# better-flow/better-flow

Measured on AMD Instinct MI355X. Metric: Mevents/s motion-compensated (warp→converged score), 1M-ev slice, 1/2/4/8 GPU, higher is better.
Workload: dtype f64

## Files before the change

better_flow_amd/csrc/bf_device_fns.h:

```cpp
#pragma once
#include <hip/hip_runtime.h>
#include <limits.h>

#include "bf_device.h"
#include "bf_kernels.h"
#include "../../include/bf_flow_color.h"
#include <math.h>
#include <math.h>

namespace bf {

__device__ __forceinline__ int trunc_x86(double v) { return bf_double_to_int_x86(v); }

__device__ __forceinline__ int trunc_scatter(double v) { return (v == v) ? __double2int_rz(v) : INT_MIN; }

__device__ __forceinline__ bool valid_px(float p) { return p > 1e-6f; }

__device__ __forceinline__ double div_10000(double x) {
    constexpr double R = 1.0 / 10000.0;
    const double q0 = x * R;
    const double r = fma(-q0, 10000.0, x);
    return fma(r, R, q0);
}
__device__ __forceinline__ float div_127(float x) {
    constexpr float R = 1.0f / 127.0f;
    const float q0 = x * R;
    const float r = fmaf(-q0, 127.0f, x);
    return fmaf(r, R, q0);
}

__device__ __forceinline__ double div_1e9(double x) {
    constexpr double R = 1.0 / 1000000000.0;
    const double q0 = x * R;
    const double r = fma(-q0, 1000000000.0, x);
    return fma(r, R, q0);
}

__device__ __forceinline__ double2 uv_from_n(double2 v) {
    const double len = hypot(v.x, v.y);
    const double speed = len / (127.0 / (double)(1000000000 / (1 * 10000)));
    double2 o;
    o.x = (len == 0) ? 0 : speed * v.x / len;
    o.y = (len == 0) ? 0 : speed * v.y / len;
    return o;
}

__device__ __forceinline__ double2 uv_from_n_nz(double2 v, double nz) {
    const double len = hypot(v.x, v.y);
    const double speed = len / (nz / (double)(1000000000 / (1 * 10000)));
    double2 o;
    o.x = (len == 0) ? 0 : speed * v.x / len;
    o.y = (len == 0) ? 0 : speed * v.y / len;
    return o;
}

__device__ __forceinline__ double pr_from_p(uint32_t fr, float prod) {
    return (double)fr - div_10000((double)prod);
}

__device__ __forceinline__ void warp_products(const WarpParams& wp, double pr_x, double pr_y, int32_t t, float2& q,
                                              double& nx, double& ny) {
    const double rx = pr_x - wp.cx, ry = pr_y - wp.cy;
    const double qx = wp.c * rx - wp.s * ry;
    const double qy = wp.s * rx + wp.c * ry;
    nx = ((-qx) * wp.div + (qx - rx)) + wp.dnx;
    ny = ((-qy) * wp.div + (qy - ry)) + wp.dny;
    const float kx = div_127((float)nx);
    const float ky = div_127((float)ny);
    const float ft = (float)t;
    q.x = kx * ft;
    q.y = ky * ft;
}

__device__ __forceinline__ int assign_pixel(const WarpParams& wp, uint32_t v, int32_t t, int scale, int x_sh, int y_sh, int wsx,
                                            int wsy, int C) {
    const uint32_t fx = v & 0xffffu, fy = v >> 16;
    float2 q;
    double nx, ny;
    warp_products(wp, (double)fx, (double)fy, t, q, nx, ny);
    const int X = trunc_scatter(pr_from_p(fx, q.x) * (double)scale + (double)x_sh);
    const int Y = trunc_scatter(pr_from_p(fy, q.y) * (double)scale + (double)y_sh);
    const int hs = scale / 2;
    if ((X >= wsx + hs) || (X < hs) || (Y >= wsy + hs) || (Y < hs)) return -1;
    return X * C + Y;
}

template <class T>
__device__ __forceinline__ T sload(const T* p) {
    static_assert(sizeof(T) % 4 == 0, "whole words");
    typedef const __attribute__((address_space(4))) uint32_t* cptr;
    const cptr src = reinterpret_cast<cptr>(reinterpret_cast<uintptr_t>(p));
    T out;
    uint32_t* dst = reinterpret_cast<uint32_t*>(&out);
#pragma unroll
    for (int i = 0; i < (int)(sizeof(T) / 4); ++i) dst[i] = src[i];
    return out;
}

__device__ __forceinline__ int wave_min(int v) {
    for (int o = 32; o > 0; o >>= 1) v = min(v, __shfl_down(v, o, 64));
    return v;
}
__device__ __forceinline__ int wave_max(int v) {
    for (int o = 32; o > 0; o >>= 1) v = max(v, __shfl_down(v, o, 64));
    return v;
}
__device__ __forceinline__ long long wave_sum(long long v) {
    for (int o = 32; o > 0; o >>= 1) v += __shfl_down(v, o, 64);
    return v;
}
__device__ __forceinline__ double wave_sum(double v) {
    for (int o = 32; o > 0; o >>= 1) v += __shfl_down(v, o, 64);
    return v;
}
__device__ __forceinline__ unsigned long long wave_sum_u64(unsigned long long v) {
    for (int o = 32; o > 0; o >>= 1) v += __shfl_down(v, o, 64);
    return v;
}
__device__ __forceinline__ uint32_t wave_max_u32(uint32_t v) {
    for (int o = 32; o > 0; o >>= 1) v = max(v, (uint32_t)__shfl_down(v, o, 64));
    return v;
}
__device__ __forceinline__ unsigned long long wave_max_u64(unsigned long long v) {
    for (int o = 32; o > 0; o >>= 1) {
        const unsigned long long w = (unsigned long long)__shfl_down((long long)v, o, 64);
        v = w > v ? w : v;
    }
    return v;
}

template <class F>
__device__ __forceinline__ void for_each_wave_key(int key, F&& f) {
    unsigned long long pending = __ballot(key >= 0);
    while (pending) {
        const int k0 = __shfl(key, __ffsll((long long)pending) - 1, 64);
        const unsigned long long same = __ballot(key == k0);
        f(k0, same);
        pending &= ~same;
    }
}

constexpr int kBoxTR = 32, kBoxTC = 64;
template <int MAXH>
__device__ __forceinline__ void box_sum_tile(const uint32_t* __restrict__ src, uint32_t* __restrict__ dst, int R, int C, int hs,
                                             int tr0, int tc0) {
    __shared__ uint32_t s_in[(kBoxTR + 2 * MAXH) * (kBoxTC + 2 * MAXH)];
    __shared__ uint32_t s_row[(kBoxTR + 2 * MAXH) * kBoxTC];
    const int IR = kBoxTR + 2 * hs, IC = kBoxTC + 2 * hs;
    for (int idx = threadIdx.x; idx < IR * IC; idx += kThreads) {
        const int lr = idx / IC, lc = idx - lr * IC;
        const int gr = tr0 - hs + lr, gc = tc0 - hs + lc;
        s_in[idx] = (gr >= 0 && gr < R && gc >= 0 && gc < C) ? src[(size_t)gr * C + gc] : 0u;
    }
    __syncthreads();
    for (int idx = threadIdx.x; idx < IR * kBoxTC; idx += kThreads) {
        const int lr = idx / kBoxTC, lc = idx % kBoxTC;
        uint32_t sum = 0;
        for (int d = 0; d <= 2 * hs; ++d) sum += s_in[lr * IC + lc + d];
        s_row[idx] = sum;
    }
    __syncthreads();
    for (int idx = threadIdx.x; idx < kBoxTR * kBoxTC; idx += kThreads) {
        const int lr = idx / kBoxTC, lc = idx % kBoxTC;
        const int gr = tr0 + lr, gc = tc0 + lc;
        if (gr >= R || gc >= C) continue;
        uint32_t sum = 0;
        for (int d = 0; d <= 2 * hs; ++d) sum += s_row[(lr + d) * kBoxTC + lc];
        dst[(size_t)gr * C + gc] = sum;
    }
}

__device__ __forceinline__ int row_bin(int row, const BinGrid& g) { return (int)__umulhi((uint32_t)row, g.mul_r); }

constexpr int kTicketGroups = 32;

constexpr int kTlLaunches = 64;
__device__ __forceinline__ void tl_stamp(unsigned long long* tl, int launch, int slot) {
#ifdef BF_TIMELINE
    if (!tl || launch >= kTlLaunches || threadIdx.x != 0) return;
// ... 662 lines not shown
```

better_flow_amd/csrc/bf_scatter.hip:

```cpp
#include <atomic>
#include <hip/hip_runtime.h>
#include <hip/hip_ext.h>
#include <limits.h>
#include <cstdlib>

#include "bf_device.h"
#include "bf_device_fns.h"
#include "bf_kernels.h"

namespace bf {

template <class T>
__device__ __forceinline__ T ld_idx(const T* base, uint32_t idx) {
    return *reinterpret_cast<const T*>(reinterpret_cast<const char*>(base) + idx * (uint32_t)sizeof(T));
}

constexpr int kMaxTileRows = 192;

struct ScatterGeo {
    int X0, Y0, L, LR;
    int zw;
};
template <bool WARP>
__device__ __forceinline__ bool event_target(const ScatterHot& hs, float2* p, uint32_t i, uint32_t v, int32_t ti,
                                             double pr_x, double pr_y, int& X, int& Y) {
    const uint32_t fx = v & 0xffffu, fy = v >> 16;
    if (WARP) {
        float2 q;
        double nx, ny;
        warp_products(hs.wp, pr_x, pr_y, ti, q, nx, ny);
        __hip_atomic_store(reinterpret_cast<unsigned long long*>(reinterpret_cast<char*>(p) + i * 8u),
                           ((unsigned long long)__float_as_uint(q.y) << 32) | (unsigned long long)__float_as_uint(q.x),
                           __ATOMIC_RELAXED, __HIP_MEMORY_SCOPE_AGENT);
        pr_x = pr_from_p(fx, q.x);
        pr_y = pr_from_p(fy, q.y);
    }
    const int s = hs.scale, hsc = hs.scale / 2;
    if (hsc > 0) {
        X = __double2int_rz(pr_x * (double)s + (double)hs.x_sh);
        Y = __double2int_rz(pr_y * (double)s + (double)hs.y_sh);
    } else {
        X = trunc_scatter(pr_x * (double)s + (double)hs.x_sh);
        Y = trunc_scatter(pr_y * (double)s + (double)hs.y_sh);
    }
    return (unsigned)(X - hsc) < (unsigned)hs.wsx && (unsigned)(Y - hsc) < (unsigned)hs.wsy;
}
__device__ __forceinline__ void overflow_add(const ScatterHot& hs, const BinScatterArgs& a, int X, int Y, unsigned long long dt) {
    const size_t kk = (size_t)X * (size_t)hs.C + (size_t)Y;
    atomicAdd(&a.ovf_plane[kk], dt);
    atomicAdd(&a.ovf_cplane[kk], 1u);
    atomicOr(&a.ovf_bits[(size_t)X * (size_t)a.ovf_pitch + (size_t)(Y >> 5) + 1], 1u << (Y & 31));
}

template <bool WARP>
__device__ __forceinline__ void scatter_event(const ScatterHot& hs, const ScatterGeo& sg, unsigned long long* s_tile,
                                              const BinScatterArgs& a, float2* p, uint32_t i, uint32_t v, int32_t ti,
                                              double pr_x, double pr_y, uint32_t& n_ovf) {
    int X, Y;
    if (!event_target<WARP>(hs, p, i, v, ti, pr_x, pr_y, X, Y)) return;
    const unsigned long long dt = (unsigned long long)((long long)ti - hs.tmin);
    const int lx = X - sg.X0, ly = Y - sg.Y0;
    if (hs.bin_ok && (unsigned)lx < (unsigned)sg.LR && (unsigned)ly < (unsigned)sg.L) {
        atomicAdd(&s_tile[__mul24(lx, sg.L) + ly], (1ull << hs.bin_tbits) + dt);
    } else {
        overflow_add(hs, a, X, Y, dt);
        ++n_ovf;
    }
}

constexpr uint32_t kNoEntry = 0xffffffffu;
template <bool WARP>
__device__ __forceinline__ uint32_t list_event(const ScatterHot& hs, const ScatterGeo& sg, const BinScatterArgs& a, float2* p,
                                               uint32_t i, uint32_t v, int32_t ti, double pr_x, double pr_y, bool take_overflow,
                                               int& row, uint32_t& n_ovf) {
    int X, Y;
    row = 0;
    if (!event_target<WARP>(hs, p, i, v, ti, pr_x, pr_y, X, Y)) return kNoEntry;
    const int lx = X - sg.X0, ly = Y - sg.Y0;
    if (hs.bin_ok && (unsigned)lx < (unsigned)sg.LR && (unsigned)ly < (unsigned)sg.L) {
        row = lx + (sg.zw ? (ly < sg.zw ? 0 : (ly >= sg.L - sg.zw ? 2 * sg.LR : sg.LR)) : 0);
        return (uint32_t)(__mul24(lx, sg.L) + ly);
    }
    if (take_overflow) {
        overflow_add(hs, a, X, Y, (unsigned long long)((long long)ti - hs.tmin));
        ++n_ovf;
    }
    return kNoEntry;
}
__device__ __forceinline__ void list_row_scan(uint32_t* s_row, int LR, uint32_t* crow, int lane) {
    uint32_t carry = 0;
    for (int r0 = 0; r0 < LR; r0 += 64) {
        const int r = r0 + lane;
        const uint32_t v = r < LR ? s_row[1 + r] : 0u;
        uint32_t incl = v;
#pragma unroll
        for (int o = 1; o < 64; o <<= 1) {
            const uint32_t u = __shfl_up(incl, o, 64);
            if (lane >= o) incl += u;
        }
        if (r < LR) {
            s_row[1 + r] = carry + incl - v;
            crow[r] = carry + incl - v;
        }
        carry += (uint32_t)__builtin_amdgcn_readlane((int)incl, 63);
    }
    if (lane == 0) crow[LR] = carry;
}
__device__ __forceinline__ void list_put(const ScatterHot& hs, const ScatterGeo& sg, const BinScatterArgs& a, uint32_t* s_row,
                                         uint32_t code, int row, int32_t ti, uint32_t LL, unsigned long long* vals,
                                         uint16_t* cidx, uint32_t& n_ovf) {
    const unsigned long long dt = (unsigned long long)((long long)ti - hs.tmin);
    const uint32_t slot = atomicAdd(&s_row[1 + row], 1u);
    if (slot < LL) {
        vals[slot] = (1ull << hs.bin_tbits) + dt;
        cidx[slot] = (uint16_t)code;
    } else {
        const int lx = row >= 2 * sg.LR ? row - 2 * sg.LR : (row >= sg.LR ? row - sg.LR : row);
        overflow_add(hs, a, sg.X0 + lx, sg.Y0 + (int)code - __mul24(lx, sg.L), dt);
        ++n_ovf;
    }
}

template <int THREADS>
__device__ __forceinline__ void flush_tile(const unsigned long long* s_tile, unsigned long long* slab, int LL, int tid) {
    const bf_u32x4* src4 = reinterpret_cast<const bf_u32x4*>(s_tile);
    for (int i = tid; i < LL / 2; i += THREADS) {
        const bf_u32x4 v = src4[i];
        asm volatile("global_store_dwordx4 %0, %1, off sc1" :: "v"(slab + 2 * i), "v"(v) : "memory");
    }
}
__device__ __forceinline__ uint32_t margin_preload(const BinScatterArgs& a, int b, uint32_t n_prev, int tid) {
    return (uint32_t)tid < n_prev ? a.mlist[(size_t)b * (size_t)a.mcap + tid] : 0xffffffffu;
}
__device__ __forceinline__ void margin_clear(const BinScatterArgs& a, int b, uint32_t n_prev, uint32_t e0, int tid, int threads) {
    if (e0 != 0xffffffffu) a.m_prev[e0] = 0ull;
    const uint32_t* lst = a.mlist + (size_t)b * (size_t)a.mcap;
    for (uint32_t i = tid + threads; i < n_prev; i += threads) a.m_prev[lst[i]] = 0ull;
}
template <int THREADS>
__device__ __forceinline__ void flush_split(const unsigned long long* s_tile, const BinScatterArgs& a, int b, int X0, int Y0, int C,
                                            uint32_t* s_mcnt , int tid) {
    const BinGrid& g = a.g;
    const bf_u32x4* src4 = reinterpret_cast<const bf_u32x4*>(s_tile);
    const int half = g.L >> 1, hD = g.D >> 1, lgh = g.lg - 1;
    unsigned long long* own = a.slabs + (size_t)b * (size_t)(g.TS * g.TSR);
    const int nown = g.TSR << lgh;
    for (int i = tid; i < nown; i += THREADS) {
        const int r = i >> lgh, q = i - (r << lgh);
        const bf_u32x4 v = src4[(r + g.D) * half + hD + q];
        asm volatile("global_store_dwordx4 %0, %1, off sc1" :: "v"(own + 2 * i), "v"(v) : "memory");
    }
    uint32_t* lst = a.mlist + (size_t)b * (size_t)a.mcap;
    const int nfull = 2 * g.D * half, nmar = nfull + g.TSR * g.D;
    const int lgD = 31 - __clz(g.D);
    for (int j = tid; j < nmar; j += THREADS) {
        int lx, lp;
        if (j < nfull) {
            const int r = (int)__umulhi((uint32_t)j, g.mul_h);
            lp = j - r * half;
            lx = r < g.D ? r : r + g.TSR;
        } else {
            const int k = j - nfull, r = k >> lgD, q = k & (g.D - 1);
            lx = g.D + r;
            lp = q < hD ? q : q + (g.TS >> 1);
        }
        const bf_u32x4 v = src4[lx * half + lp];
        const unsigned long long w0 = ((unsigned long long)v.y << 32) | v.x, w1 = ((unsigned long long)v.w << 32) | v.z;
        if (w0 | w1) {
            const uint32_t px = (uint32_t)((X0 + lx) * C + Y0 + 2 * lp);
            if (w0) {
                __hip_atomic_fetch_add(&a.m_cur[px], w0, __ATOMIC_RELAXED, __HIP_MEMORY_SCOPE_AGENT);
                lst[atomicAdd(&s_mcnt[0], 1u)] = px;
            }
            if (w1) {
                __hip_atomic_fetch_add(&a.m_cur[px + 1], w1, __ATOMIC_RELAXED, __HIP_MEMORY_SCOPE_AGENT);
                lst[atomicAdd(&s_mcnt[0], 1u)] = px + 1;
            }
        }
    }
    uint32_t arrived = 0;
    if ((tid & 63) == 0) arrived = atomicAdd(&s_mcnt[1], 1u);
    arrived = (uint32_t)__builtin_amdgcn_readfirstlane((int)arrived);
    if (arrived == THREADS / 64 - 1 && (tid & 63) == 0) a.mcount[b] = s_mcnt[0];
}
__global__ __launch_bounds__(256) void k_margin_clean(unsigned long long* mplane, const uint32_t* mlist, uint32_t* mcount, int mcap) {
    const int b = blockIdx.x;
    const uint32_t n = mcount[b];
    const uint32_t* lst = mlist + (size_t)b * (size_t)mcap;
    for (uint32_t i = threadIdx.x; i < n; i += 256) mplane[lst[i]] = 0ull;
    __syncthreads();
    if (threadIdx.x == 0) mcount[b] = 0u;
}
void launch_margin_clean(unsigned long long* mplane, const uint32_t* mlist, uint32_t* mcount, int nbins, int mcap, hipStream_t s) {
    if (nbins > 0) hipLaunchKernelGGL(k_margin_clean, dim3(nbins), dim3(256), 0, s, mplane, mlist, mcount, mcap);
}

template <bool WARP, int THREADS, int U, int FMT>
__global__ __launch_bounds__(THREADS) void k_bin_warp_scatter(const uint32_t* __restrict__ pre_bin_start, const DevState* pre_st_in,
                                                              MomentAcc* pre_acc, BinScatterArgs a) {
    constexpr bool COMPACT = FMT == 2;
    constexpr bool SPLIT = FMT == 3;
// ... 117 lines not shown
        store_state();
        if (tid < 64) list_row_scan(s_row, (g.zw ? 3 : 1) * LR, a.chdr + (size_t)b * (size_t)((g.zw ? 3 : 1) * LR + 1), tid);
        __syncthreads();
        unsigned long long* vals = a.slabs + (size_t)b * (size_t)LL;
        uint16_t* cidx = a.cidx + (size_t)b * (size_t)LL;
        if (single) {
#pragma unroll
            for (int k = 0; k < U; ++k)
                if (code[k] != kNoEntry) list_put(hs, sg, a, s_row, code[k], row[k], vt[k], (uint32_t)LL, vals, cidx, n_ovf);
        } else {
            for (base = beg; base < end; base += THREADS * U) {
                load_pass();
                previous_positions();
#pragma unroll
                for (int k = 0; k < U; ++k) {
                    const uint32_t i = base + k * THREADS + tid;
                    if (i >= end) continue;
                    int r;
                    const uint32_t cd = list_event<false>(hs, sg, a, p, i, vxy[k], vt[k], ppx[k], ppy[k], false, r, n_ovf);
                    if (cd != kNoEntry) list_put(hs, sg, a, s_row, cd, r, vt[k], (uint32_t)LL, vals, cidx, n_ovf);
                }
            }
        }
        if (n_ovf) { atomicAdd(ovf_counter(a.ovf_cur, b), n_ovf); a.ovf_cur[0] = 1u; }
        tl_stamp(a.tl, a.j, 4);
        return;
    }
    for (;;) {
#pragma unroll
        for (int k = 0; k < U; ++k) {
            const uint32_t i = base + k * THREADS + tid;
            if (i >= end) continue;
            scatter_event<WARP>(hs, sg, s_tile, a, p, i, vxy[k], vt[k], ppx[k], ppy[k], n_ovf);
        }
        base += THREADS * U;
        if (base >= end) break;
        load_pass();
        previous_positions();
    }
    if (n_ovf) { atomicAdd(ovf_counter(a.ovf_cur, b), n_ovf); a.ovf_cur[0] = 1u; }
    if (SPLIT) margin_clear(a, b, m_prev_n, m_e0, tid, THREADS);
    tl_stamp(a.tl, a.j, 2);
    __syncthreads();
    tl_stamp(a.tl, a.j, 3);
    store_state();
    if (SPLIT) flush_split<THREADS>(s_tile, a, b, X0, Y0, hs.C, s_mcnt, tid);
    else flush_tile<THREADS>(s_tile, a.slabs + (size_t)b * (size_t)LL, LL, tid);
    tl_stamp(a.tl, a.j, 4);
}

template <bool WARP, int THREADS, int U, int FMT>
__global__ __launch_bounds__(THREADS) void k_bin_warp_scatter_lean(const uint32_t* __restrict__ pre_bin_start, const DevState* pre_st_in,
                                                                   MomentAcc* , BinScatterArgs a) {
    constexpr bool COMPACT = FMT == 2;
    constexpr bool SPLIT = FMT == 3;
    extern __shared__ unsigned long long s_tile[];
    __shared__ uint32_t s_row[FMT == 2 ? 1 + 3 * kMaxTileRows : 1];
    __shared__ uint32_t s_mcnt[2];
    if (FMT == 2)
        for (int r = threadIdx.x; r <= 3 * kMaxTileRows; r += THREADS) s_row[r] = 0;
    if (SPLIT && threadIdx.x < 2) s_mcnt[threadIdx.x] = 0;
    const BinGrid& g = a.g;
    const int L = g.L, LR = g.LR, LL = g.LR * g.L;
    const int b = blockIdx.x, tid = threadIdx.x;
    const uint32_t beg = sload(pre_bin_start + b), end = sload(pre_bin_start + b + 1);
    const HotState h0 = sload(&pre_st_in->hot);
    const uint32_t m_prev_n = SPLIT ? sload(a.mcount + b) : 0u;
    const int X0 = (b / g.nbc) * g.TSR - g.D, Y0 = (b - (b / g.nbc) * g.nbc) * g.TS - g.D;
    if (!COMPACT) {
        ulonglong2* z = reinterpret_cast<ulonglong2*>(s_tile);
        for (int i = tid; i < LL / 2; i += THREADS) z[i] = make_ulonglong2(0ull, 0ull);
    }
    if (h0.done) {
        if (b == 0 && tid < kStateWords) {
            const unsigned long long state_word = reinterpret_cast<const unsigned long long*>(a.st_in)[tid];
            reinterpret_cast<unsigned long long*>(a.st_out)[tid] = state_word;
            if (a.snap) reinterpret_cast<unsigned long long*>(a.snap)[tid] = state_word;
        }
        return;
    }
    ScatterHot hs;
    hs.done = h0.done; hs.bin_tbits = h0.bin_tbits; hs.bin_ok = h0.bin_ok; hs.fmt = h0.fmt; hs.scale = h0.scale; hs.C = h0.C;
    hs.wsx = h0.wsx; hs.wsy = h0.wsy; hs.x_sh = h0.x_sh; hs.y_sh = h0.y_sh; hs.tmin = h0.tmin; hs.wp = h0.wp;
    const EvSetPtrs ev = a.sets.s[h0.cs ^ h0.flip];
    const uint32_t* __restrict__ xy = ev.xy;
    const int32_t* __restrict__ t = ev.t;
    float2* __restrict__ p = ev.p;
    const ScatterGeo sg = {X0, Y0, L, LR, FMT == 2 ? g.zw : 0};
    uint32_t n_ovf = 0;
    __syncthreads();
    uint32_t vxy[U];
    int32_t vt[U];
    float2 vp[U];
    auto load_pass = [&](uint32_t base) {
#pragma unroll
        for (int k = 0; k < U; ++k) {
            uint32_t i = base + k * THREADS + tid;
            i = i < end ? i : beg;
            vxy[k] = ld_idx(xy, i);
            vt[k] = ld_idx(t, i);
            vp[k] = ld_idx(p, i);
        }
    };
    if constexpr (COMPACT) {
        const bool single = end - beg <= (uint32_t)(THREADS * U);
        uint32_t code[U];
        int row[U];
#pragma unroll
        for (int k = 0; k < U; ++k) code[k] = kNoEntry;
        for (uint32_t base = beg; base < end; base += THREADS * U) {
            load_pass(base);
#pragma unroll
            for (int k = 0; k < U; ++k) {
                const uint32_t i = base + k * THREADS + tid;
                code[k] = kNoEntry;
                if (i >= end) continue;
                code[k] = list_event<WARP>(hs, sg, a, p, i, vxy[k], vt[k], pr_from_p(vxy[k] & 0xffffu, vp[k].x),
                                           pr_from_p(vxy[k] >> 16, vp[k].y), true, row[k], n_ovf);
                if (code[k] != kNoEntry) atomicAdd(&s_row[1 + row[k]], 1u);
            }
        }
        __syncthreads();
        if (tid < 64) list_row_scan(s_row, (g.zw ? 3 : 1) * LR, a.chdr + (size_t)b * (size_t)((g.zw ? 3 : 1) * LR + 1), tid);
        __syncthreads();
        unsigned long long* vals = a.slabs + (size_t)b * (size_t)LL;
        uint16_t* cidx = a.cidx + (size_t)b * (size_t)LL;
        if (single) {
#pragma unroll
            for (int k = 0; k < U; ++k)
                if (code[k] != kNoEntry) list_put(hs, sg, a, s_row, code[k], row[k], vt[k], (uint32_t)LL, vals, cidx, n_ovf);
        } else {
            for (uint32_t base = beg; base < end; base += THREADS * U) {
                load_pass(base);
#pragma unroll
                for (int k = 0; k < U; ++k) {
                    const uint32_t i = base + k * THREADS + tid;
                    if (i >= end) continue;
                    int r;
                    const uint32_t cd = list_event<false>(hs, sg, a, p, i, vxy[k], vt[k], pr_from_p(vxy[k] & 0xffffu, vp[k].x),
                                                          pr_from_p(vxy[k] >> 16, vp[k].y), false, r, n_ovf);
                    if (cd != kNoEntry) list_put(hs, sg, a, s_row, cd, r, vt[k], (uint32_t)LL, vals, cidx, n_ovf);
                }
            }
        }
        if (n_ovf) { atomicAdd(ovf_counter(a.ovf_cur, b), n_ovf); a.ovf_cur[0] = 1u; }
        return;
    }
    auto scatter_pass = [&](uint32_t base) {
#pragma unroll
        for (int k = 0; k < U; ++k) {
            const uint32_t i = base + k * THREADS + tid;
            if (i >= end) continue;
            scatter_event<WARP>(hs, sg, s_tile, a, p, i, vxy[k], vt[k], pr_from_p(vxy[k] & 0xffffu, vp[k].x),
                                pr_from_p(vxy[k] >> 16, vp[k].y), n_ovf);
        }
    };
    if constexpr (SPLIT) {
        const uint32_t m_e0 = margin_preload(a, b, m_prev_n, tid);
        uint32_t base = beg;
        load_pass(base);
        for (;;) {
            scatter_pass(base);
            base += THREADS * U;
            if (base >= end) break;
            load_pass(base);
        }
        if (n_ovf) { atomicAdd(ovf_counter(a.ovf_cur, b), n_ovf); a.ovf_cur[0] = 1u; }
        margin_clear(a, b, m_prev_n, m_e0, tid, THREADS);
    } else {
        for (uint32_t base = beg; base < end; base += THREADS * U) {
            load_pass(base);
            scatter_pass(base);
        }
        if (n_ovf) { atomicAdd(ovf_counter(a.ovf_cur, b), n_ovf); a.ovf_cur[0] = 1u; }
    }
    __syncthreads();
    if (SPLIT) flush_split<THREADS>(s_tile, a, b, X0, Y0, hs.C, s_mcnt, tid);
    else flush_tile<THREADS>(s_tile, a.slabs + (size_t)b * (size_t)LL, LL, tid);
}

__global__ __launch_bounds__(64) void k_finish_update(DevState* st, MomentAcc* acc, const uint32_t* ovf_prev, int j,
                                                            int cur_prev, bf_trace_rec* trace, DevState* snap, const uint32_t* lost,
                                                            unsigned long long* snap_seq, unsigned long long seq) {
    __shared__ DevState s_state;
    const int tid = threadIdx.x;
    const int done = st->hot.done, it = st->hot.it;
    const bool trip = lost && *lost != 0u && st->hot.need_rebin != 2;
    const bool apply = lost ? st->hot.pend != 0 : it < j;
    if (tid < kStateWords)
        reinterpret_cast<unsigned long long*>(&s_state)[tid] = reinterpret_cast<const unsigned long long*>(st)[tid];
    if (trip && !done) {
        __builtin_amdgcn_wave_barrier();
        if (tid == 0) { s_state.hot.need_rebin = 2; s_state.hot.redo = 1; s_state.hot.pend = 0; }
        __builtin_amdgcn_wave_barrier();
        if (tid < kStateWords)
            reinterpret_cast<unsigned long long*>(st)[tid] = reinterpret_cast<const unsigned long long*>(&s_state)[tid];
    } else if (!done && apply) {
        const uint32_t ovf = ovf_total_wave(ovf_part(ovf_prev, tid));
        unsigned long long accv[kAccPerLane];
        acc_load_wave<false, false>(acc, tid, accv);
        const unsigned long long word = acc_reduce_wave(accv);
        __builtin_amdgcn_wave_barrier();
        model_update_wave(&s_state, word, tid, 1);
        if (tid == 0) {
            model_update_rest(&s_state, trace, cur_prev, ovf);
            s_state.hot.pend = 0;
        }
        __builtin_amdgcn_wave_barrier();
        if (tid < kStateWords)
            reinterpret_cast<unsigned long long*>(st)[tid] = reinterpret_cast<const unsigned long long*>(&s_state)[tid];
    }
    if (snap && tid < kStateWords)
        reinterpret_cast<unsigned long long*>(snap)[tid] = reinterpret_cast<const unsigned long long*>(&s_state)[tid];
    if (snap_seq) {
        __threadfence_system();
        if (tid == 0) __hip_atomic_store(snap_seq, seq, __ATOMIC_RELEASE, __HIP_MEMORY_SCOPE_SYSTEM);
    }
}

template <bool HEAD, int THREADS, int U, int FMT>
static hipError_t launch_bws2(const BinScatterArgs& a, bool warp, hipStream_t s) {
    const size_t lds = FMT == 2 ? 0 : (size_t)a.g.LR * a.g.L * sizeof(unsigned long long) + 16;
    static std::atomic<unsigned long long> raised{0ull};
    const void* fns[2] = {HEAD ? reinterpret_cast<const void*>(&k_bin_warp_scatter<true, THREADS, U, FMT>)
                               : reinterpret_cast<const void*>(&k_bin_warp_scatter_lean<true, THREADS, U, FMT>),
                          HEAD ? reinterpret_cast<const void*>(&k_bin_warp_scatter<false, THREADS, U, FMT>)
                               : reinterpret_cast<const void*>(&k_bin_warp_scatter_lean<false, THREADS, U, FMT>)};
    const hipError_t e = raise_dynamic_lds(raised, fns);
    if (e != hipSuccess) return e;
    if constexpr (HEAD) {
        if (warp) launch_timed(k_bin_warp_scatter<true, THREADS, U, FMT>, dim3(a.g.nbins), dim3(THREADS), lds, s, a.bin_start, a.st_in, a.acc, a);
        else launch_timed(k_bin_warp_scatter<false, THREADS, U, FMT>, dim3(a.g.nbins), dim3(THREADS), lds, s, a.bin_start, a.st_in, a.acc, a);
    } else {
        if (warp) launch_timed(k_bin_warp_scatter_lean<true, THREADS, U, FMT>, dim3(a.g.nbins), dim3(THREADS), lds, s, a.bin_start, a.st_in, a.acc, a);
        else launch_timed(k_bin_warp_scatter_lean<false, THREADS, U, FMT>, dim3(a.g.nbins), dim3(THREADS), lds, s, a.bin_start, a.st_in, a.acc, a);
    }
    return hipSuccess;
// ... 40 lines not shown
```

better_flow_amd/csrc/bf_stencil.hip:

```cpp
#include <atomic>
#include <hip/hip_runtime.h>
#include <hip/hip_ext.h>
#include <limits.h>
#include <cstdlib>

#include "bf_device.h"
#include "bf_device_fns.h"
#include "bf_kernels.h"

namespace bf {

constexpr int kStencilSgprs = 74;
constexpr int kTileBandsBit = 0x100;

typedef unsigned int bf_u32x2 __attribute__((ext_vector_type(2)));
__device__ __forceinline__ __amdgpu_buffer_rsrc_t buf_of(const void* base) {
    return __builtin_amdgcn_make_buffer_rsrc(const_cast<void*>(base), 0, -1, 0x00020000);
}
__device__ __forceinline__ unsigned long long buf_ld_u64(__amdgpu_buffer_rsrc_t r, uint32_t thread_bytes, uint32_t uniform_bytes) {
    const bf_u32x2 v = __builtin_amdgcn_raw_buffer_load_b64(r, (int)thread_bytes, (int)uniform_bytes, 0);
    return ((unsigned long long)v.y << 32) | (unsigned long long)v.x;
}

struct K3Pre {
    const unsigned long long* slabs;
    const DevState* st;
    int R, C, D, lg, nbc, nbr, LR, L, TSR;
    uint32_t mul_r;
};
template <int HS, int MODE, int NT>
__device__ __forceinline__ void stencil_binned_body(const StencilArgs& a, const K3Pre& pre) {
    constexpr bool COMPACT = MODE == 1;
    tl_stamp(a.tl, a.tl_launch, 0);
    const HotState hs = sload(&pre.st->hot);
    tl_stamp(a.tl, a.tl_launch, 1);
    constexpr int TR = kTileR, TC = kTileC;
    constexpr int H = HS + 1;
    constexpr int PR = TR + 2 * H, PC = TC + 2 * H;
    constexpr int TH = TR + 2, TW = TC + 2;
    static_assert(TC == 64 && NT % 64 == 0, "one lane per tile column");
    constexpr int NW = NT / 64;
    constexpr int KR = (PR + NW - 1) / NW, XC = PC - 64, XE = (KR * XC + 63) / 64;
    constexpr int KT = (TH + NW - 1) / NW, XT = TW - 64;
    static_assert(KT * XT <= 64, "the time tile's extra columns fit one pass");
    __shared__ unsigned long long s_acc[PR * PC];
    __shared__ float s_time[TH * TW];
    __shared__ Sums s_red[NT / 64];
    __shared__ double s_rcp[kRcpTab];
    static_assert(NT >= kRcpTab, "one table entry per thread");
    const int R = pre.R, C = pre.C;
    const int tid = threadIdx.x;
    const double rcp_v = tid < kRcpTab ? c_rcp.v[tid] : 0.0;
    const int lane = tid & 63, wv = __builtin_amdgcn_readfirstlane(tid >> 6);
    int r0, c0;
    if (MODE != 1 && (pre.lg & kTileBandsBit)) {
        const uint32_t gx = (uint32_t)(C + TC - 1) / (uint32_t)TC, gy = (uint32_t)(R + TR - 1) / (uint32_t)TR;
        const uint32_t tile = (uint32_t)bf_rules::tile_of_block((int)blockIdx.x, (int)(gx * gy));
        const uint32_t trow = tile / gx;
        r0 = (int)trow * TR; c0 = (int)(tile - trow * gx) * TC;
    } else {
        r0 = blockIdx.y * TR; c0 = blockIdx.x * TC;
    }
    BinGrid g = a.g;
    g.D = pre.D; g.lg = pre.lg & (kTileBandsBit - 1); g.nbc = pre.nbc; g.nbr = pre.nbr; g.LR = pre.LR; g.L = pre.L; g.TSR = pre.TSR; g.mul_r = pre.mul_r;
    const int bt = hs.bin_tbits;
    const unsigned long long bm = (1ull << bt) - 1ull;
    const bool ovf = sload(a.ovf_cur) != 0;
    const int LLi = g.LR * g.L;

    constexpr bool compact = COMPACT;
    if (compact) {
        static_assert(TH * TW <= PR * PC, "the box plane fits the point plane's LDS");
        for (int idx = tid; idx < TH * TW; idx += NT) s_acc[idx] = 0ull;
        const int br_lo = row_bin(max(r0 - 1 - HS - g.D, 0), g), br_hi = min(row_bin(min(r0 + TR + HS, R - 1) + g.D, g), g.nbr - 1);
        const int bc_lo = max(c0 - 1 - HS - g.D, 0) >> g.lg, bc_hi = min((min(c0 + TC + HS, C - 1) + g.D) >> g.lg, g.nbc - 1);
        constexpr int kMaxBins = 32;
        __shared__ uint32_t s_eoff[kMaxBins + 1];
        __shared__ int2 s_ebin[kMaxBins];
        __shared__ int s_nseg;
        const int ncol = bc_hi - bc_lo + 1;
        const int zw = g.zw, nz = zw ? 3 : 1;
        const int ncand = min((br_hi - br_lo + 1) * ncol * nz, 64);
        if (tid < 64) {
            uint32_t n = 0;
            int bin = 0, r = 0, cc = 0;
            uint32_t first = 0;
            bool keep = false;
            if (tid < ncand) {
                const int bi = tid / nz, z = tid - bi * nz;
                r = bi / ncol; cc = bi - r * ncol;
                bin = (br_lo + r) * g.nbc + bc_lo + cc;
                const int top = (br_lo + r) * g.TSR - g.D;
                const int lo = min(max(r0 - 1 - HS - top, 0), g.LR), hi = min(max(r0 + TR + HS + 1 - top, 0), g.LR);
                const int left = ((bc_lo + cc) << g.lg) - g.D;
                const int z_lo = left + (z == 0 ? 0 : (z == 1 ? zw : g.L - zw)), z_hi = left + (nz == 1 ? g.L : (z == 0 ? zw : (z == 1 ? g.L - zw : g.L)));
                keep = z_hi > c0 - 1 - HS && z_lo <= c0 + TC + HS;
                if (keep) {
                    const uint32_t* crow = a.chdr + (size_t)bin * (size_t)(nz * g.LR + 1) + z * g.LR;
                    first = min(crow[lo], (uint32_t)LLi);
                    n = min(crow[hi], (uint32_t)LLi) - first;
                }
            }
            uint32_t incl = n;
#pragma unroll
            for (int o = 1; o < 64; o <<= 1) {
                const uint32_t v = __shfl_up(incl, o, 64);
                if (tid >= o) incl += v;
            }
            const unsigned long long kept = __ballot(keep);
            const int pos = __popcll(kept & ((1ull << tid) - 1ull));
            if (keep && pos < kMaxBins) {
                s_eoff[pos + 1] = incl;
// ... 43 lines not shown
        off = __mul24(gc >> g.lg, TSA) + cc;
        edge = cc < g.D || cc >= g.TS - g.D;
    };
    auto row_of = [&](int pr, bool& in, bool& edge, int& off, int& moff) {
        const int gr = r0 - H + pr;
        in = pr < PR && gr >= 0 && gr < R;
        const bool up = gr >= next_r;
        const int rr = gr - (up ? next_r : next_r - g.TSR);
        off = (up ? rp1 : rp0) + __mul24(gr, g.TS);
        edge = rr < g.D || rr >= g.TSR - g.D;
        moff = __mul24(gr, C);
    };
    unsigned long long w[KR][2], we[XE][2];
    const __amdgpu_buffer_rsrc_t slab_buf = buf_of(pre.slabs), margin_buf = buf_of(a.m_cur);
    bool c_in, c_edge;
    int c_off, c_gc;
    col_of(lane, c_in, c_edge, c_off, c_gc);
#pragma unroll
    for (int k = 0; k < KR; ++k) {
        bool r_in, r_edge;
        int r_off, r_moff;
        row_of(wv + k * NW, r_in, r_edge, r_off, r_moff);
        w[k][0] = w[k][1] = 0ull;
        if (r_in && c_in) {
            w[k][0] = buf_ld_u64(slab_buf, (uint32_t)c_off * 8u, (uint32_t)r_off * 8u);
            if (r_edge || c_edge) w[k][1] = buf_ld_u64(margin_buf, (uint32_t)c_gc * 8u, (uint32_t)r_moff * 8u);
        }
    }
#pragma unroll
    for (int x = 0; x < XE; ++x) {
        const int e = lane + 64 * x;
        bool r_in, r_edge, x_in, x_edge;
        int r_off, r_moff, x_off, x_gc;
        row_of(wv + (e / XC) * NW, r_in, r_edge, r_off, r_moff);
        col_of(64 + e % XC, x_in, x_edge, x_off, x_gc);
        we[x][0] = we[x][1] = 0ull;
        if (e < KR * XC && r_in && x_in) {
            we[x][0] = pre.slabs[(uint32_t)(r_off + x_off)];
            if (r_edge || x_edge) we[x][1] = a.m_cur[(uint32_t)(r_moff + x_gc)];
        }
    }
    if (a.check_done && hs.done) return;
#pragma unroll
    for (int k = 0; k < KR; ++k) {
        const int pr = wv + k * NW;
        if (pr < PR) s_acc[pr * PC + lane] = w[k][0] + w[k][1];
    }
#pragma unroll
    for (int x = 0; x < XE; ++x) {
        const int e = lane + 64 * x, pr = wv + (e / XC) * NW;
        if (e < KR * XC && pr < PR) s_acc[pr * PC + 64 + e % XC] = we[x][0] + we[x][1];
    }
    } else {
    static_assert(TR + 2 * H <= 32, "a tile plus halo must fit the smallest bin height (32)");
    const int bl = row_bin(max(r0 - H - g.D, 0), g), bh = row_bin(max(r0 - H + g.D, 0), g);
    const int bl_next = (bl + 1) * g.TSR, bh_next = (bh + 1) * g.TSR;
    const int rb_l0 = bl * g.nbc * LLi - (bl * g.TSR - g.D) * g.L, rb_l1 = rb_l0 + g.nbc * LLi - g.TSR * g.L;
    const int rb_h0 = bh * g.nbc * LLi - (bh * g.TSR - g.D) * g.L, rb_h1 = rb_h0 + g.nbc * LLi - g.TSR * g.L;
    auto col_of = [&](int pc, bool& in, bool& two, int& lo, int& hi) {
        const int gc = c0 - H + pc;
        in = gc >= 0 && gc < C;
        const int bcl = max(gc - g.D, 0) >> g.lg, bch = min((gc + g.D) >> g.lg, g.nbc - 1);
        lo = __mul24(bcl, LLi) - (bcl << g.lg) + g.D + gc;
        hi = __mul24(bch, LLi) - (bch << g.lg) + g.D + gc;
        two = bch > bcl;
    };
    auto row_of = [&](int pr, bool& in, bool& two, int& lo, int& hi) {
        const int gr = r0 - H + pr;
        in = pr < PR && gr >= 0 && gr < R;
        const bool l_up = max(gr - g.D, 0) >= bl_next, h_up = gr + g.D >= bh_next;
        const int brl = bl + (l_up ? 1 : 0), brh = min(bh + (h_up ? 1 : 0), g.nbr - 1);
        const int grL = __mul24(gr, g.L);
        lo = (l_up ? rb_l1 : rb_l0) + grL;
        hi = ((brh > bh) ? rb_h1 : rb_h0) + grL;
        two = brh > brl;
    };
    unsigned long long w[KR][4], we[XE][4];
    const __amdgpu_buffer_rsrc_t slab_buf = buf_of(pre.slabs);
    bool c_in, c_two;
    int c_lo, c_hi;
    col_of(lane, c_in, c_two, c_lo, c_hi);
    const uint32_t vo_lo = c_in ? (uint32_t)c_lo * 8u : 0u;
    const uint32_t vo_hi = (c_in && c_two) ? (uint32_t)c_hi * 8u : 0u;
    bool rin[KR], rtwo[KR];
#pragma unroll
    for (int k = 0; k < KR; ++k) {
        int r_lo, r_hi;
        row_of(wv + k * NW, rin[k], rtwo[k], r_lo, r_hi);
        if (rin[k]) {
            w[k][0] = buf_ld_u64(slab_buf, vo_lo, (uint32_t)r_lo * 8u);
            w[k][1] = buf_ld_u64(slab_buf, vo_hi, (uint32_t)r_lo * 8u);
            if (rtwo[k]) {
                w[k][2] = buf_ld_u64(slab_buf, vo_lo, (uint32_t)r_hi * 8u);
                w[k][3] = buf_ld_u64(slab_buf, vo_hi, (uint32_t)r_hi * 8u);
            }
        }
    }
#pragma unroll
    for (int x = 0; x < XE; ++x) {
        const int e = lane + 64 * x;
        bool r_in, r_two, x_in, x_two;
        int r_lo, r_hi, x_lo, x_hi;
        row_of(wv + (e / XC) * NW, r_in, r_two, r_lo, r_hi);
        col_of(64 + e % XC, x_in, x_two, x_lo, x_hi);
        we[x][0] = we[x][1] = we[x][2] = we[x][3] = 0ull;
        if (e < KR * XC && r_in && x_in) {
            we[x][0] = buf_ld_u64(slab_buf, (uint32_t)(r_lo + x_lo) * 8u, 0u);
            if (x_two) we[x][1] = buf_ld_u64(slab_buf, (uint32_t)(r_lo + x_hi) * 8u, 0u);
            if (r_two) we[x][2] = buf_ld_u64(slab_buf, (uint32_t)(r_hi + x_lo) * 8u, 0u);
            if (r_two && x_two) we[x][3] = buf_ld_u64(slab_buf, (uint32_t)(r_hi + x_hi) * 8u, 0u);
        }
    }
    if (a.check_done && hs.done) return;
#pragma unroll
    for (int k = 0; k < KR; ++k) {
        const int pr = wv + k * NW;
        if (pr < PR) {
            unsigned long long sum = 0ull;
            if (rin[k]) {
                sum = w[k][0] + w[k][1];
                if (rtwo[k]) sum += w[k][2] + w[k][3];
            }
            s_acc[pr * PC + lane] = sum;
        }
    }
#pragma unroll
    for (int x = 0; x < XE; ++x) {
        const int e = lane + 64 * x, pr = wv + (e / XC) * NW;
        if (e < KR * XC && pr < PR) s_acc[pr * PC + 64 + e % XC] = (we[x][0] + we[x][1]) + (we[x][2] + we[x][3]);
    }
    }
    __shared__ uint32_t s_bits[(TH + 2 * HS) * 4];
    if (ovf) {
        for (int i = tid; i < (TH + 2 * HS) * 4; i += NT) {
            const int gr = r0 - 1 - HS + (i >> 2);
            s_bits[i] = (gr >= 0 && gr < R) ? a.ovf_bits[(size_t)gr * (size_t)a.ovf_pitch + (size_t)((c0 >> 5) + (i & 3))] : 0u;
        }
    }
    if (tid < kRcpTab) s_rcp[tid] = rcp_v;
    tl_stamp(a.tl, a.tl_launch, 2);
    __syncthreads();
    tl_stamp(a.tl, a.tl_launch, 3);
    auto box_at = [&](const int tr, const int tc) {
        if (compact) return s_acc[tr * TW + tc];
        unsigned long long pk = 0;
#pragma unroll
        for (int da = 0; da <= 2 * HS; ++da)
#pragma unroll
            for (int db = 0; db <= 2 * HS; ++db) pk += s_acc[(tr + da) * PC + (tc + db)];
        return pk;
    };
    auto time_px = [&](const int tr, const int tc, const unsigned long long pk) {
        const int idx = tr * TW + tc;
        const int gr = r0 - 1 + tr, gc = c0 - 1 + tc;
        float tv = 0.f;
        if (gr >= 0 && gr < R && gc >= 0 && gc < C) {
            unsigned long long acc = pk & bm;
            uint32_t cacc = (uint32_t)(pk >> bt);
            bool box_dirty = false;
            if (ovf) {
                const int ps = tc + 31 - HS;
                uint32_t any = 0;
#pragma unroll
                for (int da = 0; da <= 2 * HS; ++da) {
                    const uint32_t* rw = &s_bits[(tr + da) * 4 + (ps >> 5)];
                    const unsigned long long w2 = ((unsigned long long)rw[1] << 32) | rw[0];
                    any |= (uint32_t)(w2 >> (ps & 31)) & ((1u << (2 * HS + 1)) - 1u);
                }
                box_dirty = any != 0;
            }
            if (box_dirty) {
#pragma unroll
                for (int da = -HS; da <= HS; ++da)
#pragma unroll
                    for (int db = -HS; db <= HS; ++db) {
                        const int pr_ = gr + da, pc_ = gc + db;
                        if (pr_ >= 0 && pr_ < R && pc_ >= 0 && pc_ < C) {
                            acc += a.plane[(uint32_t)(__mul24(pr_, C) + pc_)];
                            cacc += a.cplane[(uint32_t)(__mul24(pr_, C) + pc_)];
                        }
                    }
            }
            tv = time_from_sums(cacc, (long long)acc, a.tmin, s_rcp);
        }
        s_time[idx] = tv;
    };
    constexpr int LW = TH % NW;
    if constexpr (COMPACT) {
#pragma unroll
        for (int k = 0; k < KT; ++k) {
            const int tr = wv + k * NW;
            if (tr < TH) time_px(tr, lane, box_at(tr, lane));
        }
    } else {
        const int nrows = (LW == 0 || wv < LW) ? KT : KT - 1;
        const int rbeg = (LW == 0 || wv < LW) ? wv * KT : LW * KT + (wv - LW) * (KT - 1);
        unsigned long long hsum[KT + 2 * HS];
#pragma unroll
        for (int j = 0; j < KT + 2 * HS; ++j) {
            hsum[j] = 0ull;
            if (j < nrows + 2 * HS) {
#pragma unroll
                for (int db = 0; db <= 2 * HS; ++db) hsum[j] += s_acc[(rbeg + j) * PC + (lane + db)];
            }
        }
#pragma unroll
        for (int i = 0; i < KT; ++i) {
            if (i < nrows) {
                unsigned long long pk = 0;
#pragma unroll
                for (int da = 0; da <= 2 * HS; ++da) pk += hsum[i + da];
                time_px(rbeg + i, lane, pk);
            }
        }
    }
    if constexpr (LW != 0 && NW - LW >= XT && TH <= 64) {
        if (wv >= LW && wv < LW + XT && lane < TH) time_px(lane, 64 + (wv - LW), box_at(lane, 64 + (wv - LW)));
    } else {
        if (lane < KT * XT) {
            const int tr = wv + (lane / XT) * NW;
            if (tr < TH) time_px(tr, 64 + lane % XT, box_at(tr, 64 + lane % XT));
        }
    }
    __syncthreads();
    tl_stamp(a.tl, a.tl_launch, 4);
    const bool do_zero = a.zero_plane && sload(a.ovf_prev) != 0;
    static_assert((size_t)PR * PC >= (size_t)(NT / 64) * 192, "the reduction's scratch fits the accumulator plane");
    stencil_tail<TR, TC, NT, false>(a, s_time, s_red, r0, c0, do_zero, reinterpret_cast<double*>(s_acc));
}

#define BF_K3_PRE_PARAMS const unsigned long long* p_slabs, const DevState* p_st, int p_R, int p_C, int p_D, int p_lg, \
                          int p_nbc, int p_nbr, int p_LR, int p_L, int p_TSR, uint32_t p_mul_r
#define BF_K3_PRE_VALUE K3Pre{p_slabs, p_st, p_R, p_C, p_D, p_lg, p_nbc, p_nbr, p_LR, p_L, p_TSR, p_mul_r}
template <int HS, int MODE, int NT>
__global__ __launch_bounds__(NT) void k_stencil_binned(BF_K3_PRE_PARAMS, StencilArgs a) {
    stencil_binned_body<HS, MODE, NT>(a, BF_K3_PRE_VALUE);
}
template <int HS, int MODE, int NT>
__global__ __launch_bounds__(NT) __attribute__((amdgpu_num_sgpr(kStencilSgprs))) void k_stencil_binned_full(BF_K3_PRE_PARAMS, StencilArgs a) {
    stencil_binned_body<HS, MODE, NT>(a, BF_K3_PRE_VALUE);
}


void launch_stencil_binned(const StencilArgs& a, dim3 tiles, hipStream_t s, int n_cus) {
    const bool full = bf_rules::stencil_capped((long long)tiles.x * tiles.y, n_cus);
    const bool bands = a.tile_bands && bf_rules::stencil_mode(a.compact) != 1;
    const dim3 grid = bands ? dim3(tiles.x * tiles.y) : tiles;
#define BF_K3_PRE a.slabs, a.st, a.R, a.C, a.g.D, a.g.lg | (bands ? kTileBandsBit : 0), a.g.nbc, a.g.nbr, a.g.LR, a.g.L, a.g.TSR, a.g.mul_r
#define BF_K3(HS_)                                                                                                  \
    if (full) {                                                                                                     \
        if (a.compact == 3) launch_timed(k_stencil_binned_full<HS_, 2, kThreads>, grid, dim3(kThreads), 0, s, BF_K3_PRE, a);   \
        else if (a.compact) launch_timed(k_stencil_binned_full<HS_, 1, kThreads>, grid, dim3(kThreads), 0, s, BF_K3_PRE, a);   \
        else launch_timed(k_stencil_binned_full<HS_, 0, kThreads>, grid, dim3(kThreads), 0, s, BF_K3_PRE, a);                  \
    } else if (a.compact == 3) launch_timed(k_stencil_binned<HS_, 2, kThreads>, grid, dim3(kThreads), 0, s, BF_K3_PRE, a);     \
    else if (a.compact) launch_timed(k_stencil_binned<HS_, 1, kThreads>, grid, dim3(kThreads), 0, s, BF_K3_PRE, a);            \
    else launch_timed(k_stencil_binned<HS_, 0, kThreads>, grid, dim3(kThreads), 0, s, BF_K3_PRE, a)
    switch (bf_rules::stencil_half_scale(a.scale)) {
        case 0: BF_K3(0); break;
        case 1: BF_K3(1); break;
        case 2: BF_K3(2); break;
        case 3: BF_K3(3); break;
        default: BF_K3(4); break;
    }
#undef BF_K3
#undef BF_K3_PRE
}

}
```

Measured before the change: 213.7.

## Reload kernel args late from kernarg segment and pin uniform values in SGPRs

```diff
diff --git a/better_flow_amd/csrc/bf_device_fns.h b/better_flow_amd/csrc/bf_device_fns.h
--- a/better_flow_amd/csrc/bf_device_fns.h
+++ b/better_flow_amd/csrc/bf_device_fns.h
@@ -95,6 +95,24 @@
 #pragma unroll
     for (int i = 0; i < (int)(sizeof(T) / 4); ++i) dst[i] = src[i];
     return out;
+}
+
+template <class A>
+__device__ __forceinline__ const A* late_args(unsigned offset) {
+    uintptr_t k = reinterpret_cast<uintptr_t>(__builtin_amdgcn_kernarg_segment_ptr());
+    asm volatile("" : "+s"(k));
+    return reinterpret_cast<const A*>(k + offset);
+}
+
+template <class T>
+__device__ __forceinline__ T* as_global(T* p) {
+    typedef __attribute__((address_space(1))) T* gptr;
+    return (T*)reinterpret_cast<gptr>(reinterpret_cast<uintptr_t>(p));
+}
+
+template <class T>
+__device__ __forceinline__ void uniform_here(T& v) {
+    asm volatile("" : "+s"(v));
 }
 
 __device__ __forceinline__ int wave_min(int v) {
diff --git a/better_flow_amd/csrc/bf_scatter.hip b/better_flow_amd/csrc/bf_scatter.hip
--- a/better_flow_amd/csrc/bf_scatter.hip
+++ b/better_flow_amd/csrc/bf_scatter.hip
@@ -45,14 +45,27 @@
     }
     return (unsigned)(X - hsc) < (unsigned)hs.wsx && (unsigned)(Y - hsc) < (unsigned)hs.wsy;
 }
+constexpr unsigned kScatterArgsOffset = 24;
+static_assert(alignof(BinScatterArgs) == 8, "the argument struct starts right behind the three leading pointers");
+template <bool LATE>
 __device__ __forceinline__ void overflow_add(const ScatterHot& hs, const BinScatterArgs& a, int X, int Y, unsigned long long dt) {
+    unsigned long long* ovf_plane = a.ovf_plane;
+    uint32_t *ovf_cplane = a.ovf_cplane, *ovf_bits = a.ovf_bits;
+    int ovf_pitch = a.ovf_pitch;
+    if constexpr (LATE) {
+        const BinScatterArgs* la = late_args<BinScatterArgs>(kScatterArgsOffset);
+        ovf_plane = as_global(sload(&la->ovf_plane));
+        ovf_cplane = as_global(sload(&la->ovf_cplane));
+        ovf_bits = as_global(sload(&la->ovf_bits));
+        ovf_pitch = sload(&la->ovf_pitch);
+    }
     const size_t kk = (size_t)X * (size_t)hs.C + (size_t)Y;
-    atomicAdd(&a.ovf_plane[kk], dt);
-    atomicAdd(&a.ovf_cplane[kk], 1u);
-    atomicOr(&a.ovf_bits[(size_t)X * (size_t)a.ovf_pitch + (size_t)(Y >> 5) + 1], 1u << (Y & 31));
-}
-
-template <bool WARP>
+    atomicAdd(&ovf_plane[kk], dt);
+    atomicAdd(&ovf_cplane[kk], 1u);
+    atomicOr(&ovf_bits[(size_t)X * (size_t)ovf_pitch + (size_t)(Y >> 5) + 1], 1u << (Y & 31));
+}
+
+template <bool WARP, bool LATE = false>
 __device__ __forceinline__ void scatter_event(const ScatterHot& hs, const ScatterGeo& sg, unsigned long long* s_tile,
                                               const BinScatterArgs& a, float2* p, uint32_t i, uint32_t v, int32_t ti,
                                               double pr_x, double pr_y, uint32_t& n_ovf) {
@@ -63,7 +76,7 @@
     if (hs.bin_ok && (unsigned)lx < (unsigned)sg.LR && (unsigned)ly < (unsigned)sg.L) {
         atomicAdd(&s_tile[__mul24(lx, sg.L) + ly], (1ull << hs.bin_tbits) + dt);
     } else {
-        overflow_add(hs, a, X, Y, dt);
+        overflow_add<LATE>(hs, a, X, Y, dt);
         ++n_ovf;
     }
 }
@@ -82,7 +95,7 @@
         return (uint32_t)(__mul24(lx, sg.L) + ly);
     }
     if (take_overflow) {
-        overflow_add(hs, a, X, Y, (unsigned long long)((long long)ti - hs.tmin));
+        overflow_add<false>(hs, a, X, Y, (unsigned long long)((long long)ti - hs.tmin));
         ++n_ovf;
     }
     return kNoEntry;
@@ -116,7 +129,7 @@
         cidx[slot] = (uint16_t)code;
     } else {
         const int lx = row >= 2 * sg.LR ? row - 2 * sg.LR : (row >= sg.LR ? row - sg.LR : row);
-        overflow_add(hs, a, sg.X0 + lx, sg.Y0 + (int)code - __mul24(lx, sg.L), dt);
+        overflow_add<false>(hs, a, sg.X0 + lx, sg.Y0 + (int)code - __mul24(lx, sg.L), dt);
         ++n_ovf;
     }
 }
@@ -400,6 +413,12 @@
     ScatterHot hs;
     hs.done = h0.done; hs.bin_tbits = h0.bin_tbits; hs.bin_ok = h0.bin_ok; hs.fmt = h0.fmt; hs.scale = h0.scale; hs.C = h0.C;
     hs.wsx = h0.wsx; hs.wsy = h0.wsy; hs.x_sh = h0.x_sh; hs.y_sh = h0.y_sh; hs.tmin = h0.tmin; hs.wp = h0.wp;
+    constexpr bool DIET = WARP && FMT == 0 && U >= 4;
+    if constexpr (DIET) {
+        uniform_here(hs.wp.dnx); uniform_here(hs.wp.dny); uniform_here(hs.wp.cx); uniform_here(hs.wp.cy);
+        uniform_here(hs.wp.div); uniform_here(hs.wp.c); uniform_here(hs.wp.s);
+        uniform_here(hs.x_sh); uniform_here(hs.y_sh);
+    }
     const EvSetPtrs ev = a.sets.s[h0.cs ^ h0.flip];
     const uint32_t* __restrict__ xy = ev.xy;
     const int32_t* __restrict__ t = ev.t;
@@ -410,11 +429,13 @@
     uint32_t vxy[U];
     int32_t vt[U];
     float2 vp[U];
+    const uint32_t last = end > beg ? end - 1 : beg;
     auto load_pass = [&](uint32_t base) {
 #pragma unroll
         for (int k = 0; k < U; ++k) {
             uint32_t i = base + k * THREADS + tid;
-            i = i < end ? i : beg;
+            if constexpr (DIET) i = min(i, last);
+            else i = i < end ? i : beg;
             vxy[k] = ld_idx(xy, i);
             vt[k] = ld_idx(t, i);
             vp[k] = ld_idx(p, i);
@@ -465,12 +486,14 @@
         return;
     }
     auto scatter_pass = [&](uint32_t base) {
+        static_assert((THREADS & (THREADS - 1)) == 0, "slots by a shift");
+        const int nslot = ((int)(end - base) - tid + (THREADS - 1)) >> (31 - __builtin_clz(THREADS));
 #pragma unroll
         for (int k = 0; k < U; ++k) {
             const uint32_t i = base + k * THREADS + tid;
-            if (i >= end) continue;
-            scatter_event<WARP>(hs, sg, s_tile, a, p, i, vxy[k], vt[k], pr_from_p(vxy[k] & 0xffffu, vp[k].x),
-                                pr_from_p(vxy[k] >> 16, vp[k].y), n_ovf);
+            if (DIET ? k >= nslot : i >= end) continue;
+            scatter_event<WARP, DIET>(hs, sg, s_tile, a, p, i, vxy[k], vt[k], pr_from_p(vxy[k] & 0xffffu, vp[k].x),
+                                      pr_from_p(vxy[k] >> 16, vp[k].y), n_ovf);
         }
     };
     if constexpr (SPLIT) {
diff --git a/better_flow_amd/csrc/bf_stencil.hip b/better_flow_amd/csrc/bf_stencil.hip
--- a/better_flow_amd/csrc/bf_stencil.hip
+++ b/better_flow_amd/csrc/bf_stencil.hip
@@ -28,6 +28,8 @@
     int R, C, D, lg, nbc, nbr, LR, L, TSR;
     uint32_t mul_r;
 };
+constexpr unsigned kStencilArgsOffset = 56;
+static_assert(sizeof(K3Pre) == kStencilArgsOffset && alignof(StencilArgs) == 8, "the argument struct starts right behind the leading arguments");
 template <int HS, int MODE, int NT>
 __device__ __forceinline__ void stencil_binned_body(const StencilArgs& a, const K3Pre& pre) {
     constexpr bool COMPACT = MODE == 1;
@@ -237,20 +239,27 @@
     col_of(lane, c_in, c_two, c_lo, c_hi);
     const uint32_t vo_lo = c_in ? (uint32_t)c_lo * 8u : 0u;
     const uint32_t vo_hi = (c_in && c_two) ? (uint32_t)c_hi * 8u : 0u;
-    bool rin[KR], rtwo[KR];
+    static_assert(KR <= 8, "row bits");
+    uint32_t rowbits = 0;
 #pragma unroll
     for (int k = 0; k < KR; ++k) {
+        bool r_in, r_two;
         int r_lo, r_hi;
-        row_of(wv + k * NW, rin[k], rtwo[k], r_lo, r_hi);
-        if (rin[k]) {
+        row_of(wv + k * NW, r_in, r_two, r_lo, r_hi);
+        if (r_in) {
+            rowbits |= 1u << k;
             w[k][0] = buf_ld_u64(slab_buf, vo_lo, (uint32_t)r_lo * 8u);
             w[k][1] = buf_ld_u64(slab_buf, vo_hi, (uint32_t)r_lo * 8u);
-            if (rtwo[k]) {
+            if (r_two) {
+                rowbits |= 0x100u << k;
                 w[k][2] = buf_ld_u64(slab_buf, vo_lo, (uint32_t)r_hi * 8u);
                 w[k][3] = buf_ld_u64(slab_buf, vo_hi, (uint32_t)r_hi * 8u);
             }
         }
     }
+    int wv_s = wv;
+    uniform_here(rowbits);
+    uniform_here(wv_s);
 #pragma unroll
     for (int x = 0; x < XE; ++x) {
         const int e = lane + 64 * x;
@@ -269,12 +278,12 @@
     if (a.check_done && hs.done) return;
 #pragma unroll
     for (int k = 0; k < KR; ++k) {
-        const int pr = wv + k * NW;
+        const int pr = wv_s + k * NW;
         if (pr < PR) {
             unsigned long long sum = 0ull;
-            if (rin[k]) {
+            if (rowbits & (1u << k)) {
                 sum = w[k][0] + w[k][1];
-                if (rtwo[k]) sum += w[k][2] + w[k][3];
+                if (rowbits & (0x100u << k)) sum += w[k][2] + w[k][3];
             }
             s_acc[pr * PC + lane] = sum;
         }
@@ -325,14 +334,17 @@
                 box_dirty = any != 0;
             }
             if (box_dirty) {
+                const StencilArgs* la = late_args<StencilArgs>(kStencilArgsOffset);
+                const unsigned long long* const plane = as_global(sload(&la->plane));
+                const uint32_t* const cplane = as_global(sload(&la->cplane));
 #pragma unroll
                 for (int da = -HS; da <= HS; ++da)
 #pragma unroll
                     for (int db = -HS; db <= HS; ++db) {
                         const int pr_ = gr + da, pc_ = gc + db;
                         if (pr_ >= 0 && pr_ < R && pc_ >= 0 && pc_ < C) {
-                            acc += a.plane[(uint32_t)(__mul24(pr_, C) + pc_)];
-                            cacc += a.cplane[(uint32_t)(__mul24(pr_, C) + pc_)];
+                            acc += plane[(uint32_t)(__mul24(pr_, C) + pc_)];
+                            cacc += cplane[(uint32_t)(__mul24(pr_, C) + pc_)];
                         }
                     }
             }
@@ -377,11 +389,17 @@
             if (tr < TH) time_px(tr, 64 + lane % XT, box_at(tr, 64 + lane % XT));
         }
     }
+    StencilArgs ta = sload(late_args<StencilArgs>(kStencilArgsOffset));
+    ta.st = as_global(ta.st); ta.acc = as_global(ta.acc); ta.acc_zero = as_global(ta.acc_zero);
+    ta.ovf_cur = as_global(ta.ovf_cur); ta.ovf_prev = as_global(ta.ovf_prev); ta.ovf_next = as_global(ta.ovf_next);
+    ta.zero_plane = as_global(ta.zero_plane); ta.zero_cplane = as_global(ta.zero_cplane); ta.zero_bits = as_global(ta.zero_bits);
+    ta.ticket = as_global(ta.ticket); ta.st_rw = as_global(ta.st_rw); ta.snap = as_global(ta.snap);
+    ta.trace = as_global(ta.trace); ta.tl = as_global(ta.tl);
     __syncthreads();
-    tl_stamp(a.tl, a.tl_launch, 4);
-    const bool do_zero = a.zero_plane && sload(a.ovf_prev) != 0;
+    tl_stamp(ta.tl, ta.tl_launch, 4);
+    const bool do_zero = ta.zero_plane && sload(ta.ovf_prev) != 0;
     static_assert((size_t)PR * PC >= (size_t)(NT / 64) * 192, "the reduction's scratch fits the accumulator plane");
-    stencil_tail<TR, TC, NT, false>(a, s_time, s_red, r0, c0, do_zero, reinterpret_cast<double*>(s_acc));
+    stencil_tail<TR, TC, NT, false>(ta, s_time, s_red, r0, c0, do_zero, reinterpret_cast<double*>(s_acc));
 }
 
 #define BF_K3_PRE_PARAMS const unsigned long long* p_slabs, const DevState* p_st, int p_R, int p_C, int p_D, int p_lg, \
```

New measurement: 218.5, median of 6. +2.2%, better.
